# noamteyssier/ibu

Measured on AMD Instinct MI355X. Metric: records/s, fused 2-bit decode+encode of 24-byte IBU records (HBM-resident), higher is better.
Workload: dtype u64

## Files before the change

ibu_amd/csrc/device.cpp:

```cpp
#include <stdlib.h>
#include <stddef.h>
#include <string.h>

#include <chrono>

#include <cstddef>
#include "bgzf_plan.hpp"
#include "ctx.hpp"

using namespace ibu;

namespace {

int32_t check_ctx(const ibu_ctx* ctx) {
  if (!ctx) return err_arg("ctx is NULL");
  hipError_t e = hipSetDevice(ctx->device);
  if (e != hipSuccess) return hip_fail(e, "hipSetDevice");
  return IBU_OK;
}
int32_t check_lens(uint32_t bc_len, uint32_t umi_len) {
  if (bc_len == 0 || bc_len > 32) return err_bc_len(bc_len);
  if (umi_len == 0 || umi_len > 32) return err_umi_len(umi_len);
  return IBU_OK;
}
// ... 131 lines not shown
  if (strcmp(key, "bgzf_range_bytes") == 0) {
    if (value < 0) return err_arg("bgzf_range_bytes must be >= 0");
    ctx->bgzf_range_bytes_opt = (size_t)value;
    return IBU_OK;
  }
  if (strcmp(key, "bgzf_device") == 0) {
    if (value != 0 && value != 1) return err_arg("bgzf_device must be 0 or 1");
    ctx->bgzf_device = (int)value;
    return IBU_OK;
  }
  if (strcmp(key, "bgzf_stream_ahead") == 0) {
    if (value != 0 && value != 1) return err_arg("bgzf_stream_ahead must be 0 or 1");
    ctx->bgzf_stream_ahead = (int)value;
    return IBU_OK;
  }
  if (strcmp(key, "load_piece_delay_ms") == 0) {
    if (value < 0 || value > 10000) return err_arg("load_piece_delay_ms must be 0 .. 10000");
    ctx->load_piece_delay_ms = (uint32_t)value;
    return IBU_OK;
  }
  if (strcmp(key, "release_staging") == 0) {
    if (value != 1) return err_arg("release_staging must be 1");
    if (ctx->stage_lent) return err_arg("an open ibu_stream_open_path stream loads through the staging: close it first");
    IBU_HIP(hipSetDevice(ctx->device));
    for (hipStream_t q : ctx->inflate_streams)
      if (q) IBU_HIP(hipStreamSynchronize(q));
    if (ctx->d_inflate_stage) IBU_HIP(hipFree(ctx->d_inflate_stage));
    ctx->d_inflate_stage = nullptr;
    ctx->inflate_stage_bytes = 0;
    for (int b = 0; b < 2; ++b) {
      if (ctx->d_range_buf[b]) IBU_HIP(hipFree(ctx->d_range_buf[b]));
      ctx->d_range_buf[b] = nullptr;
      ctx->range_buf_bytes[b] = 0;
    }
    return IBU_OK;
  }
  if (strcmp(key, "sort_pull_streams") == 0) {
    if (value != 0 && value != 1) return err_arg("sort_pull_streams must be 0 or 1");
    ctx->force_pull_streams = (int)value;
    return IBU_OK;
  }
  if (strcmp(key, "peer_access") == 0) {
    if (value != 0 && value != 1) return err_arg("peer_access must be 0 or 1");
    ctx->peer_access = (int)value;
    return IBU_OK;
  }
  if (strcmp(key, "numa") == 0) {
    if (value != 0 && value != 1) return err_arg("numa must be 0 (off) or 1 (auto)");
    ctx->numa_mode = (int)value;
    return IBU_OK;
  }
  if (strcmp(key, "trace_rows") == 0) {
    ctx->cfg.trace_rows = value != 0;
    return IBU_OK;
  }
  if (strcmp(key, "base_order") == 0) {
    if (value != IBU_BASE_ORDER_LSB_FIRST && value != IBU_BASE_ORDER_MSB_FIRST) return err_arg("base_order must be 0 (LSB first) or 1 (MSB first)");
    ctx->cfg.base_order = (uint32_t)value;
    return IBU_OK;
  }
  return err_arg("unknown option key");
}
extern "C" int32_t ibu_ctx_device(const ibu_ctx_t* ctx) { return ctx ? ctx->device : -1; }
extern "C" int32_t ibu_ctx_numa(const ibu_ctx_t* ctx, ibu_numa_info_t* out) {
  if (!ctx || !out) return err_arg("ctx or out is NULL");
  memset(out, 0, sizeof *out);
  out->mode = ctx->numa_mode;
  out->node = ctx->place.node;
  out->usable_cpus = ctx->place.ncpus;
  out->ring_node = ctx->ring.slots ? ctx->ring.node : -1;
  out->ring_placed = ctx->ring.slots && ctx->ring.placed ? 1 : 0;
  snprintf(out->pci_bus_id, sizeof out->pci_bus_id, "%s", ctx->pci_bus_id);
  snprintf(out->cpulist, sizeof out->cpulist, "%s", ctx->place.cpulist);
  return IBU_OK;
}
extern "C" void* ibu_ctx_stream(const ibu_ctx_t* ctx) { return ctx ? ctx->stream : nullptr; }
extern "C" int32_t ibu_ctx_synchronize(ibu_ctx_t* ctx, void* stream) {
  int32_t rc = check_ctx(ctx);
  if (rc) return rc;
  IBU_HIP(hipStreamSynchronize(pick_stream(ctx, stream)));
  return IBU_OK;
}
extern "C" int32_t ibu_device_alloc(ibu_ctx_t* ctx, size_t bytes, void** d_ptr) {
  int32_t rc = check_ctx(ctx);
  if (rc) return rc;
  if (!d_ptr) return err_arg("d_ptr is NULL");
  return ibu::ctx_alloc(ctx, bytes, d_ptr);
}
static int32_t alloc_probed_impl(ibu_ctx_t* ctx, size_t bytes, uint32_t tries, void** d_ptr, ibu_alloc_probe_t* report, double alloc_budget_ms,
                                 double* slow_ms);
static uint32_t probe_tries_for(const ibu_ctx* ctx, size_t bytes) {
  const int t = ctx->cfg.alloc_probe_tries;
  if (t == 1) return 1;
  if (t > 1) return bytes >= ((size_t)256 << 20) ? (uint32_t)t : 1u;
  if (bytes < ((size_t)1 << 30)) return 1;
  size_t free_b = 0, total_b = 0;
  if (hipMemGetInfo(&free_b, &total_b) != hipSuccess) { (void)hipGetLastError(); return 1; }
  const size_t fit = free_b / bytes;
  return fit < 3 ? 1u : (fit < 4 ? (uint32_t)fit : 4u);
}
hipError_t ibu::ctx_malloc(ibu_ctx* ctx, void** p, size_t bytes) {
  hipError_t e = hipMalloc(p, bytes ? bytes : 16);
  if (e == hipErrorOutOfMemory && ctx->loser_free.joinable()) {
    (void)hipGetLastError();
    ctx->loser_free.join();
    e = hipMalloc(p, bytes ? bytes : 16);
// ... 849 lines not shown
```

ibu_amd/csrc/k_decode.hip:

```cpp
#include "kcommon.hpp"
#include "kernels.h"

namespace ibu {

constexpr bool dword_len(int len) { return len > 0 && (len & 3) == 0; }
#ifndef IBU_DECODE_GEN_NT
#define IBU_DECODE_GEN_NT 1
#endif
template <int BC, int UM>
constexpr int dec_nt() {
#ifdef IBU_DECODE_NT
  return IBU_DECODE_NT;
#else
  if (BC == 0 && UM == 0) return IBU_DECODE_GEN_NT;
  return (dword_len(BC) && dword_len(UM) && BC + UM >= 20) ? 2 : 1;
#endif
}

template <int NT>
struct DecRegs {
  u32x4 v[3 * NT];
  __device__ __forceinline__ void load(const uint8_t* src) {
#pragma unroll
    for (int k = 0; k < 3 * NT; ++k) v[k] = ld16(src + 1024 * k);
  }
};

template <int BC, int UM, bool MSB>
__device__ __forceinline__ void decode_tile(uint8_t* tile, const DecRegs<dec_nt<BC, UM>()>& a, u32 t, u32 bc_len, u32 umi_len,
                                            uint8_t* bc_out, uint8_t* umi_out, u64* idx_out, u32 lane) {
  constexpr int kDecodeNT = dec_nt<BC, UM>(), kDecLoads = 3 * kDecodeNT, kDecRecs = kTileRecs * kDecodeNT;
  wave_lds_fence();
#pragma unroll
  for (int k = 0; k < kDecLoads; ++k) *reinterpret_cast<u32x4*>(tile + 1024 * k + 16 * lane) = a.v[k];
  wave_lds_fence();
  if constexpr (MSB) {
    rev_pairs_tile<kDecodeNT>(tile, 24, 0, bc_len, lane);
    rev_pairs_tile<kDecodeNT>(tile, 24, 8, umi_len, lane);
    wave_lds_fence();
  }
  u32* const stream_bc = reinterpret_cast<u32*>(tile + kTileBytes * kDecodeNT);
  u32* const stream_umi = reinterpret_cast<u32*>(tile + kTileBytes * kDecodeNT + (BC == 0 ? stream_bytes(kDecodeNT) : 0));
  if (bc_out) expand_field<BC, kDecodeNT>(tile, 24, 0, bc_len, bc_out + (size_t)t * kDecRecs * bc_len, lane, stream_bc);
  if (umi_out) expand_field<UM, kDecodeNT>(tile, 24, 8, umi_len, umi_out + (size_t)t * kDecRecs * umi_len, lane, stream_umi);
  if (idx_out) {
#pragma unroll
    for (int j = 0; j < kDecodeNT; ++j) {
      const u32 c = lane + 64 * j;
      u64 i0 = *reinterpret_cast<const u64*>(tile + (2 * c) * 24 + 16);
      u64 i1 = *reinterpret_cast<const u64*>(tile + (2 * c + 1) * 24 + 16);
      u32x4 o; o.x = (u32)i0; o.y = (u32)(i0 >> 32); o.z = (u32)i1; o.w = (u32)(i1 >> 32);
      st16(reinterpret_cast<uint8_t*>(idx_out) + (size_t)t * (8 * kDecRecs) + 16 * c, o);
    }
  }
}

#ifndef IBU_DECODE_GEN_WAVES
#define IBU_DECODE_GEN_WAVES 6
#endif
template <int BC, int UM, bool MSB>
constexpr int dec_waves() {
  if (BC == 0 || UM == 0) return (BC == 12 || UM == 12) ? 5 : IBU_DECODE_GEN_WAVES;
  if (dec_nt<BC, UM>() > 1) return (BC == 12 || UM == 12) ? 4 : (MSB ? 4 : 5);
  return MSB ? 6 : 7;
}
template <int BC, int UM, bool MSB>
__global__ void __launch_bounds__(kBlock, (dec_waves<BC, UM, MSB>()))
ibu_k_decode(const uint8_t* __restrict__ recs, u32 ntiles, u32 bc_len, u32 umi_len,
             uint8_t* __restrict__ bc_out, uint8_t* __restrict__ umi_out, u64* __restrict__ idx_out) {
  constexpr int kDecBytes = kTileBytes * dec_nt<BC, UM>();
  constexpr int kWaveLds = kDecBytes + ((BC == 0) + (UM == 0)) * (int)stream_bytes(dec_nt<BC, UM>());
  __shared__ __attribute__((aligned(16))) uint8_t lds[kWavesPerBlock * kWaveLds];
  const u32 lane = threadIdx.x & (kWave - 1);
  const u32 wib = threadIdx.x >> 6;
  uint8_t* tile = lds + wib * kWaveLds;
  const TileRange tr = tile_range(ntiles, wib);
  const u32 nwaves = tr.stride;
  u32 t = tr.t;
  ntiles = tr.end;
  if (t >= ntiles) return;
  if (BC > 0) bc_len = BC;
  if (UM > 0) umi_len = UM;

  DecRegs<dec_nt<BC, UM>()> a, b;
  a.load(recs + (size_t)t * kDecBytes + 16 * lane);
  for (;;) {
    u32 tn = t + nwaves;
    bool more = tn < ntiles;
    b.load(recs + (size_t)(more ? tn : t) * kDecBytes + 16 * lane);
    decode_tile<BC, UM, MSB>(tile, a, t, bc_len, umi_len, bc_out, umi_out, idx_out, lane);
    if (!more) break;
    t = tn;
    tn = t + nwaves;
    more = tn < ntiles;
    a.load(recs + (size_t)(more ? tn : t) * kDecBytes + 16 * lane);
    decode_tile<BC, UM, MSB>(tile, b, t, bc_len, umi_len, bc_out, umi_out, idx_out, lane);
    if (!more) break;
    t = tn;
  }
}

#ifndef IBU_UNPACK_GEN_NT
#define IBU_UNPACK_GEN_NT 2
#endif
constexpr int unpack_nt(int len) { return len == 0 ? IBU_UNPACK_GEN_NT : len <= 16 ? 4 : 2; }
constexpr int unpack_waves(int len) { return len == 0 ? 6 : len <= 16 ? 6 : 8; }
template <int LEN, bool MSB>
__global__ void __launch_bounds__(kBlock, unpack_waves(LEN))
ibu_k_unpack(const u64* __restrict__ codes, u32 ntiles , u32 len, uint8_t* __restrict__ out) {
  constexpr int NT = unpack_nt(LEN);
  constexpr int kWaveLds = 1024 * NT + (LEN == 0 ? (int)stream_bytes(NT) : 0);
  __shared__ __attribute__((aligned(16))) uint8_t lds[kWavesPerBlock * kWaveLds];
  const u32 lane = threadIdx.x & (kWave - 1);
  const u32 wib = threadIdx.x >> 6;
  uint8_t* tile = lds + wib * kWaveLds;
  if (LEN > 0) len = LEN;
  const uint8_t* base = reinterpret_cast<const uint8_t*>(codes) + 16 * lane;
  struct Regs { u32x4 v[NT]; };
  sweep_tiles<Regs>(
      tile_range(ntiles, wib),
      [&](Regs& g, u32 t) {
#pragma unroll
        for (int k = 0; k < NT; ++k) g.v[k] = ld16(base + ((size_t)t * NT + k) * 1024);
      },
      [&](const Regs& g, u32 t) {
        wave_lds_fence();
#pragma unroll
        for (int k = 0; k < NT; ++k)
          *reinterpret_cast<u32x4*>(tile + 1024 * k + 16 * lane) = MSB ? rev_pairs_x2(g.v[k], len) : g.v[k];
        wave_lds_fence();
        expand_field<LEN, NT>(tile, 8, 0, len, out + (size_t)t * NT * kTileRecs * len, lane, reinterpret_cast<u32*>(tile + 1024 * NT));
      });
}

__device__ __forceinline__ void unpack_row_bytes(u64 code, u32 len, u32 msb, uint8_t* out) {
  if (msb) code = rev_pairs(code, len);
  for (u32 i = 0; i < len; ++i) {
    const u32 half = (u32)(code >> (i & 16u ? 32 : 0));
    out[i] = (uint8_t)__builtin_amdgcn_ubfe(kPool, 8 * __builtin_amdgcn_ubfe(half, 2 * (i & 15u), 2), 8);
  }
}
extern "C" __global__ void ibu_k_decode_tail(const u64* __restrict__ recs, u64 row0, u64 n, u32 bc_len,
                                             u32 umi_len, u32 msb, uint8_t* bc_out, uint8_t* umi_out, u64* idx_out) {
  const u64 i = row0 + (u64)blockIdx.x * blockDim.x + threadIdx.x;
  if (i >= n) return;
  if (bc_out) unpack_row_bytes(recs[3 * i], bc_len, msb, bc_out + i * bc_len);
  if (umi_out) unpack_row_bytes(recs[3 * i + 1], umi_len, msb, umi_out + i * umi_len);
  if (idx_out) idx_out[i] = recs[3 * i + 2];
}
extern "C" __global__ void ibu_k_unpack_tail(const u64* codes, u64 row0, u64 n, u32 len, u32 msb, uint8_t* out) {
  const u64 i = row0 + (u64)blockIdx.x * blockDim.x + threadIdx.x;
  if (i >= n) return;
  unpack_row_bytes(codes[i], len, msb, out + i * len);
}

typedef void (*DecFn)(const uint8_t*, u32, u32, u32, uint8_t*, uint8_t*, u64*);
template <int B, int U, bool M>
static constexpr DecFn dec_entry() { return ibu_k_decode<len_of_mode(B), len_of_mode(U), M>; }
#define IBU_DEC_ROW(B, M) {dec_entry<B, 0, M>(), dec_entry<B, 1, M>(), dec_entry<B, 2, M>(), dec_entry<B, 3, M>(), dec_entry<B, 4, M>()}
#define IBU_DEC_TABLE(M) {IBU_DEC_ROW(0, M), IBU_DEC_ROW(1, M), IBU_DEC_ROW(2, M), IBU_DEC_ROW(3, M), IBU_DEC_ROW(4, M)}
static const DecFn kDecTable[2][kNumLenModes][kNumLenModes] = {IBU_DEC_TABLE(false), IBU_DEC_TABLE(true)};
template <int B, int U>
static constexpr int dec_recs() { return kTileRecs * dec_nt<len_of_mode(B), len_of_mode(U)>(); }
#define IBU_DEC_RECS_ROW(B) {dec_recs<B, 0>(), dec_recs<B, 1>(), dec_recs<B, 2>(), dec_recs<B, 3>(), dec_recs<B, 4>()}
static const int kDecRecsTable[kNumLenModes][kNumLenModes] = {IBU_DEC_RECS_ROW(0), IBU_DEC_RECS_ROW(1), IBU_DEC_RECS_ROW(2),
                                                              IBU_DEC_RECS_ROW(3), IBU_DEC_RECS_ROW(4)};

hipError_t launch_decode(const LaunchCfg& cfg, const void* recs, size_t n, uint32_t bc_len, uint32_t umi_len,
                         uint8_t* bc, uint8_t* umi, uint64_t* idx, hipStream_t st) {
  (void)hipGetLastError();
  if (n == 0) return hipSuccess;
  const Span sp[4] = {{recs, 24}, {bc, bc_len}, {umi, umi_len}, {idx, 8}};
  const size_t kDecRecs = (size_t)kDecRecsTable[mode_of_len(bc_len)][mode_of_len(umi_len)];
  const RowSplit rs = split_rows(cfg, sp, 4, n, kDecRecs);
  if (rs.head)
    hipLaunchKernelGGL(ibu_k_decode_tail, dim3(tail_grid(rs.head)), dim3(256), 0, st, (const u64*)recs, (u64)0,
                       (u64)rs.head, bc_len, umi_len, cfg.base_order, bc, umi, (u64*)idx);
  if (rs.main) {
    const u32 ntiles = (u32)(rs.main / kDecRecs);
    const int mb = mode_of_len(bc_len), mu = mode_of_len(umi_len);
    const int mo = cfg.base_order ? 1 : 0;
    const DecFn fn = kDecTable[mo][mb][mu];
    static std::atomic<int> occ[2][kNumLenModes][kNumLenModes];
    hipLaunchKernelGGL(fn, dim3(grid_for(ntiles, cfg.cus, resident_blocks<kBlock>(cfg, fn, 0, &occ[mo][mb][mu]))), dim3(kBlock), 0,
                       st, adv((const uint8_t*)recs, 24 * rs.head), ntiles, bc_len, umi_len, adv(bc, rs.head * bc_len),
                       adv(umi, rs.head * umi_len), adv((u64*)idx, 8 * rs.head));
  }
  if (rs.head + rs.main < n)
    hipLaunchKernelGGL(ibu_k_decode_tail, dim3(tail_grid(n - rs.head - rs.main)), dim3(256), 0, st, (const u64*)recs,
                       (u64)(rs.head + rs.main), (u64)n, bc_len, umi_len, cfg.base_order, bc, umi, (u64*)idx);
  return hipGetLastError();
}

typedef void (*UnpFn)(const u64*, u32, u32, uint8_t*);
#define IBU_UNP_ROW(M) {ibu_k_unpack<len_of_mode(0), M>, ibu_k_unpack<len_of_mode(1), M>, ibu_k_unpack<len_of_mode(2), M>, \
                        ibu_k_unpack<len_of_mode(3), M>, ibu_k_unpack<len_of_mode(4), M>}
static const UnpFn kUnpTable[2][kNumLenModes] = {IBU_UNP_ROW(false), IBU_UNP_ROW(true)};

hipError_t launch_unpack(const LaunchCfg& cfg, const uint64_t* codes, size_t n, uint32_t len, uint8_t* out,
                         hipStream_t st) {
  (void)hipGetLastError();
  if (n == 0) return hipSuccess;
  const Span sp[2] = {{codes, 8}, {out, len}};
  const size_t tile_recs = (size_t)kTileRecs * unpack_nt(len_of_mode(mode_of_len(len)));
  const RowSplit rs = split_rows(cfg, sp, 2, n, tile_recs);
  if (rs.head)
    hipLaunchKernelGGL(ibu_k_unpack_tail, dim3(tail_grid(rs.head)), dim3(256), 0, st, (const u64*)codes, (u64)0, (u64)rs.head,
                       len, cfg.base_order, out);
  if (rs.main) {
    const u32 ntiles = (u32)(rs.main / tile_recs);
    const int m = mode_of_len(len), mo = cfg.base_order ? 1 : 0;
    static std::atomic<int> occ[2][kNumLenModes];
    hipLaunchKernelGGL(kUnpTable[mo][m], dim3(grid_for(ntiles, cfg.cus, resident_blocks<kBlock>(cfg, kUnpTable[mo][m], 0, &occ[mo][m]))),
                       dim3(kBlock), 0, st, adv((const u64*)codes, 8 * rs.head), ntiles, len, adv(out, rs.head * len));
  }
  if (rs.head + rs.main < n)
    hipLaunchKernelGGL(ibu_k_unpack_tail, dim3(tail_grid(n - rs.head - rs.main)), dim3(256), 0, st, (const u64*)codes,
                       (u64)(rs.head + rs.main), (u64)n, len, cfg.base_order, out);
  return hipGetLastError();
}

}
```

ibu_amd/csrc/k_encode.hip:

```cpp
#include "kcommon.hpp"
#include "kernels.h"

namespace ibu {

#ifndef IBU_ENCODE_MINWAVES
#define IBU_ENCODE_MINWAVES 6
#endif
#ifndef IBU_ENCODE_GEN_MINWAVES
#define IBU_ENCODE_GEN_MINWAVES 4
#endif
constexpr int encode_minwaves(int bc, int um) {
  if (bc == 0 || um == 0) return IBU_ENCODE_GEN_MINWAVES;
  return (bc <= 16 && um <= 16) ? IBU_ENCODE_MINWAVES : 4;
}
__host__ __device__ constexpr u32 enc_field_lds(int spec_len, u32 len) { return spec_len > 0 ? 128u * len : 32u * len + kStreamPad; }
template <int BC, int UM>
constexpr int enc_nt() {
#ifdef IBU_ENCODE_NT
  return (BC > 0 && UM > 0 && (BC & 3) == 0 && (UM & 3) == 0) ? IBU_ENCODE_NT : 1;
#else
  return 1;
#endif
}
#ifndef IBU_ENCODE_NT2_MINWAVES
#define IBU_ENCODE_NT2_MINWAVES 5
#endif
template <int BC, int UM>
constexpr int enc_waves() { return enc_nt<BC, UM>() > 1 ? IBU_ENCODE_NT2_MINWAVES : encode_minwaves(BC, UM); }

template <int BC, int UM, bool MSB>
__global__ void __launch_bounds__(kBlock, (enc_waves<BC, UM>()))
ibu_k_encode(const uint8_t* __restrict__ bc_in, const uint8_t* __restrict__ umi_in,
             const u64* __restrict__ idx_in, u64 first_index, u64 row_base, u32 ntiles, u32 bc_len, u32 umi_len,
             u32 wave_lds_bytes, uint8_t* __restrict__ recs, u64* __restrict__ status) {
  constexpr int NT = enc_nt<BC, UM>(), kRecs = kTileRecs * NT;
  extern __shared__ __attribute__((aligned(16))) uint8_t dyn_lds[];
  const u32 lane = threadIdx.x & (kWave - 1);
  const u32 wib = threadIdx.x >> 6;
  if (BC > 0) bc_len = BC;
  if (UM > 0) umi_len = UM;
  uint8_t* area = dyn_lds + wib * wave_lds_bytes;
  uint8_t* asc_bc = area;
  uint8_t* asc_umi = area + enc_field_lds(BC, bc_len) * NT;
  const TileRange tr = tile_range(ntiles, wib);
  const u32 nwaves = tr.stride;
  u32 t = tr.t;
  ntiles = tr.end;
  if (t >= ntiles) return;
  const uint8_t* idx_src = idx_in ? reinterpret_cast<const uint8_t*>(idx_in) + 16 * lane : bc_in;
  const size_t idx_tile = idx_in ? 1024 * NT : 0, idx_sub = idx_in ? 1024 : 0;

  AsciiStage<BC, NT> sb;
  AsciiStage<UM, NT> su;
  u32x4 vi[NT];
  sb.issue(bc_in + (size_t)t * kRecs * bc_len, bc_len, lane);
  su.issue(umi_in + (size_t)t * kRecs * umi_len, umi_len, lane);
#pragma unroll
  for (int j = 0; j < NT; ++j) vi[j] = ld16(idx_src + (size_t)t * idx_tile + j * idx_sub);
  BadRows bad;
  for (;;) {
    const size_t row0 = (size_t)t * kRecs;
    wave_lds_fence();
    const bool okcb = sb.land(asc_bc, bc_len, lane), okcu = su.land(asc_umi, umi_len, lane);
    const bool chunks_ok = okcb && okcu;
    u64 ix[NT][2];
#pragma unroll
    for (int j = 0; j < NT; ++j) {
      ix[j][0] = ((u64)vi[j].y << 32) | vi[j].x;
      ix[j][1] = ((u64)vi[j].w << 32) | vi[j].z;
      if (!idx_in) { ix[j][0] = first_index + row0 + 128 * j + 2 * lane; ix[j][1] = ix[j][0] + 1; }
    }
    const u32 tn = t + nwaves;
    const bool more = tn < ntiles;
    const u32 tp = more ? tn : t;
    sb.issue(bc_in + (size_t)tp * kRecs * bc_len, bc_len, lane);
    su.issue(umi_in + (size_t)tp * kRecs * umi_len, umi_len, lane);
#pragma unroll
    for (int j = 0; j < NT; ++j) vi[j] = ld16(idx_src + (size_t)tp * idx_tile + j * idx_sub);
    wave_lds_fence();
    u64 b[NT][2], u[NT][2];
#pragma unroll
    for (int j = 0; j < NT; ++j)
#pragma unroll
      for (int h = 0; h < 2; ++h) {
        const u32 r = 128 * j + 2 * lane + h;
        bool okb = true, oku = true;
#if IBU_PROBE == 1
        b[j][h] = *reinterpret_cast<const u32*>(asc_bc + r * bc_len);
        u[j][h] = *reinterpret_cast<const u32*>(asc_umi + r * umi_len);
#elif IBU_PROBE == 2
        b[j][h] = row0 + r;
        u[j][h] = b[j][h] * 3;
#else
        b[j][h] = pack_row<BC>(asc_bc, r, bc_len, okb);
        u[j][h] = pack_row<UM>(asc_umi, r, umi_len, oku);
        if constexpr (BC == 0 || UM == 0) {
          if (__ballot(!chunks_ok) != 0) {
            if constexpr (BC == 0) b[j][h] = pack_row_bytes(bc_in + (row0 + r) * bc_len, bc_len, okb);
            if constexpr (UM == 0) u[j][h] = pack_row_bytes(umi_in + (row0 + r) * umi_len, umi_len, oku);
          }
        }
#endif
        if (!okb) b[j][h] = 0;
        if (!oku) u[j][h] = 0;
        bad.note(!(okb && oku), row_base + row0 + r);
      }
    wave_lds_fence();
#pragma unroll
    for (int j = 0; j < NT; ++j) {
      u64* r = reinterpret_cast<u64*>(area + (128 * j + 2 * lane) * 24);
      r[0] = b[j][0]; r[1] = u[j][0]; r[2] = ix[j][0]; r[3] = b[j][1]; r[4] = u[j][1]; r[5] = ix[j][1];
    }
    wave_lds_fence();
    if constexpr (MSB) {
      rev_pairs_tile<NT>(area, 24, 0, bc_len, lane);
      rev_pairs_tile<NT>(area, 24, 8, umi_len, lane);
      wave_lds_fence();
    }
    uint8_t* dst = recs + (size_t)t * (kTileBytes * NT) + 16 * lane;
#pragma unroll
    for (int k = 0; k < 3 * NT; ++k) st16(dst + 1024 * k, *reinterpret_cast<const u32x4*>(area + 1024 * k + 16 * lane));
    if (!more) break;
    t = tn;
  }
  bad.flush(status);
}

constexpr int pack_nt(int len) { return (len > 0 && len <= 16) ? 2 : 1; }
template <int LEN, bool MSB, int GNT = 1, int RND = 0>
__global__ void __launch_bounds__(kBlock, LEN == 0 ? (RND >= 7 ? 5 : (GNT >= 4 || RND >= 5) ? 6 : 8) : LEN <= 12 ? 5 : 4)
ibu_k_pack(const uint8_t* __restrict__ in, u64 row_base, u32 ntiles , u32 len, u64* __restrict__ codes,
           u64* __restrict__ status) {
  constexpr int NT = LEN > 0 ? pack_nt(LEN) : GNT, kRows = kTileRecs * NT;
  constexpr u32 kWaveLds = LEN > 0 ? (u32)(kRows * LEN) : (u32)(256 * (RND > 0 ? RND : 4)) + kStreamPad;
  __shared__ __attribute__((aligned(16))) uint8_t lds[kWavesPerBlock * kWaveLds];
  const u32 lane = threadIdx.x & (kWave - 1);
  const u32 wib = threadIdx.x >> 6;
  uint8_t* asc = lds + wib * kWaveLds;
  const TileRange tr = tile_range(ntiles, wib);
  const u32 nwaves = tr.stride;
  u32 t = tr.t;
  ntiles = tr.end;
  if (LEN > 0) len = LEN;
  if (t >= ntiles) return;
  AsciiStage<LEN, NT, RND> sv;
  sv.issue(in + (size_t)t * kRows * len, len, lane);
  BadRows bad;
  for (;;) {
    const size_t row0 = (size_t)t * kRows;
    wave_lds_fence();
    const bool chunks_ok = sv.land(asc, len, lane);
    const u32 tn = t + nwaves;
    const bool more = tn < ntiles;
    sv.issue(in + (size_t)(more ? tn : t) * kRows * len, len, lane);
    wave_lds_fence();
#pragma unroll
    for (int j = 0; j < NT; ++j) {
      const u32 r = 128 * j + 2 * lane;
      bool ok0 = true, ok1 = true;
      u64 v0 = pack_row<LEN>(asc, r, len, ok0);
      u64 v1 = pack_row<LEN>(asc, r + 1, len, ok1);
      if constexpr (LEN == 0) {
        if (__ballot(!chunks_ok) != 0) {
          v0 = pack_row_bytes(in + (row0 + r) * len, len, ok0);
          v1 = pack_row_bytes(in + (row0 + r + 1) * len, len, ok1);
        }
      }
      if constexpr (MSB) { v0 = rev_pairs(v0, len); v1 = rev_pairs(v1, len); }
      if (!ok0) v0 = 0;
      if (!ok1) v1 = 0;
      bad.note(!ok0, row_base + row0 + r);
      bad.note(!ok1, row_base + row0 + r + 1);
      u32x4 o; o.x = (u32)v0; o.y = (u32)(v0 >> 32); o.z = (u32)v1; o.w = (u32)(v1 >> 32);
      st16(reinterpret_cast<uint8_t*>(codes) + (row0 + 128 * j) * 8 + 16 * lane, o);
    }
    if (!more) break;
    t = tn;
  }
  bad.flush(status);
}

extern "C" __global__ void ibu_k_encode_tail(const uint8_t* bc_in, const uint8_t* umi_in, const u64* idx_in,
                                             u64 first_index, u64 row0, u64 n, u32 bc_len, u32 umi_len, u32 msb,
                                             u64* __restrict__ recs, u64* status) {
  const u64 i = row0 + (u64)blockIdx.x * blockDim.x + threadIdx.x;
  if (i >= n) return;
  bool okb = true, oku = true;
  u64 b = pack_row_bytes(bc_in + i * bc_len, bc_len, okb);
  u64 u = pack_row_bytes(umi_in + i * umi_len, umi_len, oku);
  if (msb) { b = rev_pairs(b, bc_len); u = rev_pairs(u, umi_len); }
  if (!okb) b = 0;
  if (!oku) u = 0;
  if (!(okb && oku)) { atomicMin(&status[0], i); atomicAdd(&status[1], 1ull); }
  recs[3 * i] = b; recs[3 * i + 1] = u; recs[3 * i + 2] = idx_in ? idx_in[i] : first_index + i;
}
extern "C" __global__ void ibu_k_pack_tail(const uint8_t* in, u64 row0, u64 n, u32 len, u32 msb, u64* codes, u64* status) {
  const u64 i = row0 + (u64)blockIdx.x * blockDim.x + threadIdx.x;
  if (i >= n) return;
  bool ok = true;
  u64 v = pack_row_bytes(in + i * len, len, ok);
  if (msb) v = rev_pairs(v, len);
  if (!ok) { v = 0; atomicMin(&status[0], i); atomicAdd(&status[1], 1ull); }
  codes[i] = v;
}

typedef void (*EncFn)(const uint8_t*, const uint8_t*, const u64*, u64, u64, u32, u32, u32, u32, uint8_t*, u64*);
template <int B, int U, bool M>
static constexpr EncFn enc_entry() { return ibu_k_encode<len_of_mode(B), len_of_mode(U), M>; }
#define IBU_ENC_ROW(B, M) {enc_entry<B, 0, M>(), enc_entry<B, 1, M>(), enc_entry<B, 2, M>(), enc_entry<B, 3, M>(), enc_entry<B, 4, M>()}
#define IBU_ENC_TABLE(M) {IBU_ENC_ROW(0, M), IBU_ENC_ROW(1, M), IBU_ENC_ROW(2, M), IBU_ENC_ROW(3, M), IBU_ENC_ROW(4, M)}
static const EncFn kEncTable[2][kNumLenModes][kNumLenModes] = {IBU_ENC_TABLE(false), IBU_ENC_TABLE(true)};
template <int B, int U>
static constexpr int enc_nt_of() { return enc_nt<len_of_mode(B), len_of_mode(U)>(); }
#define IBU_ENC_NT_ROW(B) {enc_nt_of<B, 0>(), enc_nt_of<B, 1>(), enc_nt_of<B, 2>(), enc_nt_of<B, 3>(), enc_nt_of<B, 4>()}
static const int kEncNtTable[kNumLenModes][kNumLenModes] = {IBU_ENC_NT_ROW(0), IBU_ENC_NT_ROW(1), IBU_ENC_NT_ROW(2),
                                                            IBU_ENC_NT_ROW(3), IBU_ENC_NT_ROW(4)};

hipError_t launch_encode(const LaunchCfg& cfg, const uint8_t* bc, const uint8_t* umi, const uint64_t* idx,
                         uint64_t first_index, size_t n, uint32_t bc_len, uint32_t umi_len, void* recs,
                         uint64_t* status, hipStream_t st) {
  (void)hipGetLastError();
  if (n == 0) return hipSuccess;
  const Span sp[4] = {{recs, 24}, {bc, bc_len}, {umi, umi_len}, {idx, 8}};
  const int mb = mode_of_len(bc_len), mu = mode_of_len(umi_len);
  const u32 nt = (u32)kEncNtTable[mb][mu];
  const size_t tile_recs = (size_t)kTileRecs * nt;
  const RowSplit rs = split_rows(cfg, sp, 4, n, tile_recs);
  if (rs.head)
    hipLaunchKernelGGL(ibu_k_encode_tail, dim3(tail_grid(rs.head)), dim3(256), 0, st, bc, umi, (const u64*)idx, (u64)first_index,
                       (u64)0, (u64)rs.head, bc_len, umi_len, cfg.base_order, (u64*)recs, (u64*)status);
  if (rs.main) {
    const u32 ntiles = (u32)(rs.main / tile_recs);
    u32 wave_lds = (enc_field_lds(len_of_mode(mb), bc_len) + enc_field_lds(len_of_mode(mu), umi_len)) * nt;
    if (wave_lds < (u32)kTileBytes * nt) wave_lds = kTileBytes * nt;
    const int mo = cfg.base_order ? 1 : 0;
    const EncFn fn = kEncTable[mo][mb][mu];
    static std::atomic<int> occ[2][33][33];
    const int nb = resident_blocks<kBlock>(cfg, fn, wave_lds * kWavesPerBlock, &occ[mo][bc_len][umi_len]);
    hipLaunchKernelGGL(fn, dim3(grid_for(ntiles, cfg.cus, nb)), dim3(kBlock), wave_lds * kWavesPerBlock, st,
                       adv(bc, rs.head * bc_len), adv(umi, rs.head * umi_len), adv((const u64*)idx, 8 * rs.head),
                       (u64)(first_index + rs.head), (u64)rs.head, ntiles, bc_len, umi_len, wave_lds,
                       adv((uint8_t*)recs, 24 * rs.head), (u64*)status);
  }
  if (rs.head + rs.main < n)
    hipLaunchKernelGGL(ibu_k_encode_tail, dim3(tail_grid(n - rs.head - rs.main)), dim3(256), 0, st, bc, umi, (const u64*)idx,
                       (u64)first_index, (u64)(rs.head + rs.main), (u64)n, bc_len, umi_len, cfg.base_order, (u64*)recs, (u64*)status);
  return hipGetLastError();
}

typedef void (*PackFn)(const uint8_t*, u64, u32, u32, u64*, u64*);
#define IBU_PACK_ROW(M) {nullptr , ibu_k_pack<len_of_mode(1), M>, ibu_k_pack<len_of_mode(2), M>, \
                         ibu_k_pack<len_of_mode(3), M>, ibu_k_pack<len_of_mode(4), M>}
static const PackFn kPackTable[2][kNumLenModes] = {IBU_PACK_ROW(false), IBU_PACK_ROW(true)};
struct PackShape { int nt, rounds; };
static inline PackShape pack_shape(uint32_t len) {
  const int nt = len <= 8 ? 4 : 2;
  return {nt, (int)(len * nt + 7) / 8};
}
template <bool M>
static PackFn pack_gen_entry(int nt, int rounds) {
  switch (nt * 10 + rounds) {
    case 41: return ibu_k_pack<0, M, 4, 1>;
    case 42: return ibu_k_pack<0, M, 4, 2>;
    case 43: return ibu_k_pack<0, M, 4, 3>;
    case 44: return ibu_k_pack<0, M, 4, 4>;
    case 23: return ibu_k_pack<0, M, 2, 3>;
    case 24: return ibu_k_pack<0, M, 2, 4>;
    case 25: return ibu_k_pack<0, M, 2, 5>;
    case 26: return ibu_k_pack<0, M, 2, 6>;
    case 27: return ibu_k_pack<0, M, 2, 7>;
    default: return ibu_k_pack<0, M, 2, 8>;
  }
}

hipError_t launch_pack(const LaunchCfg& cfg, const uint8_t* in, size_t n, uint32_t len, uint64_t* codes,
                       uint64_t* status, hipStream_t st) {
  (void)hipGetLastError();
  if (n == 0) return hipSuccess;
  const Span sp[2] = {{in, len}, {codes, 8}};
  const int m = mode_of_len(len), mo = cfg.base_order ? 1 : 0;
  const PackShape shape = m ? PackShape{pack_nt(len_of_mode(m)), 0} : pack_shape(len);
  const size_t tile_rows = (size_t)kTileRecs * shape.nt;
  const RowSplit rs = split_rows(cfg, sp, 2, n, tile_rows);
  if (rs.head)
    hipLaunchKernelGGL(ibu_k_pack_tail, dim3(tail_grid(rs.head)), dim3(256), 0, st, in, (u64)0, (u64)rs.head, len, cfg.base_order,
                       (u64*)codes, (u64*)status);
  if (rs.main) {
    const u32 ntiles = (u32)(rs.main / tile_rows);
    const PackFn fn = m ? kPackTable[mo][m] : (mo ? pack_gen_entry<true>(shape.nt, shape.rounds) : pack_gen_entry<false>(shape.nt, shape.rounds));
    static std::atomic<int> occ[2][kNumLenModes], occ_gen[2][33];
    std::atomic<int>* oc = m ? &occ[mo][m] : &occ_gen[mo][len];
    hipLaunchKernelGGL(fn, dim3(grid_for(ntiles, cfg.cus, resident_blocks<kBlock>(cfg, fn, 0, oc))),
                       dim3(kBlock), 0, st, adv(in, rs.head * len), (u64)rs.head, ntiles, len, adv((u64*)codes, 8 * rs.head),
                       (u64*)status);
  }
// ... 8 lines not shown
```

ibu_amd/csrc/kcommon.hpp:

```cpp
#pragma once
#include <hip/hip_runtime.h>
#include <stdint.h>
#include <stdio.h>
#include <stdlib.h>

#include "kernels.h"

namespace ibu {

typedef unsigned int u32;
typedef unsigned long long u64;
typedef u32 u32x4 __attribute__((ext_vector_type(4)));
typedef u32 u32x2 __attribute__((ext_vector_type(2)));

static constexpr int kWave = 64;
#ifndef IBU_BLOCK
#define IBU_BLOCK 256
#endif
static constexpr int kBlock = IBU_BLOCK;
static constexpr int kWavesPerBlock = kBlock / kWave;
static constexpr int kTileRecs = 128;
static constexpr int kTileBytes = kTileRecs * 24;
static constexpr u32 kPool = 0x54474341u;

static constexpr int kNumLenModes = 5;
__host__ __device__ constexpr int len_of_mode(int m) { return m == 1 ? 8 : m == 2 ? 12 : m == 3 ? 16 : m == 4 ? 32 : 0; }
static inline int mode_of_len(uint32_t len) {
  switch (len) {
    case 8: return 1;
    case 12: return 2;
    case 16: return 3;
    case 32: return 4;
    default: return 0;
  }
}

#ifndef IBU_XCD_REMAP
#define IBU_XCD_REMAP 1
#endif
__device__ __forceinline__ u32 logical_block() {
#if IBU_XCD_REMAP
  const u32 nb = gridDim.x;
  if (nb & 7u) return blockIdx.x;
  return (blockIdx.x & 7u) * (nb >> 3) + (blockIdx.x >> 3);
#else
  return blockIdx.x;
#endif
}

#ifndef IBU_XCD_STATIC
#define IBU_XCD_STATIC 1
#endif
struct TileRange { u32 t, stride, end; };
#ifndef IBU_XCD_SUB
#define IBU_XCD_SUB 1
#endif
__device__ __forceinline__ TileRange tile_range(u32 ntiles, u32 wib) {
#if IBU_XCD_STATIC
  if ((gridDim.x & 7u) == 0 && gridDim.x >= 8u * IBU_XCD_SUB) {
    const u32 parts = 8u * IBU_XCD_SUB;
    const u32 tpp = (ntiles + parts - 1) / parts;
    const u32 xcd = blockIdx.x & 7u, lb = blockIdx.x >> 3, nbx = gridDim.x >> 3;
    const u32 sub = lb % IBU_XCD_SUB, part = xcd * IBU_XCD_SUB + sub;
    const u32 nb_sub = (nbx - sub + IBU_XCD_SUB - 1) / IBU_XCD_SUB;
    const u32 t0 = part * tpp, t1 = t0 + tpp < ntiles ? t0 + tpp : ntiles;
    return {t0 + (lb / IBU_XCD_SUB) * (u32)kWavesPerBlock + wib, nb_sub * (u32)kWavesPerBlock, t0 < ntiles ? t1 : 0u};
  }
#endif
  return {logical_block() * (u32)kWavesPerBlock + wib, gridDim.x * (u32)kWavesPerBlock, ntiles};
}

template <class Regs, class Load, class Body>
__device__ __forceinline__ void sweep_tiles(const TileRange tr, Load load, Body body) {
  u32 t = tr.t;
  if (t >= tr.end) return;
  Regs a, b;
  load(a, t);
  for (;;) {
    u32 tn = t + tr.stride;
    bool more = tn < tr.end;
    load(b, more ? tn : t);
    body(a, t);
    if (!more) break;
    t = tn;
    tn = t + tr.stride;
    more = tn < tr.end;
    load(a, more ? tn : t);
    body(b, t);
    if (!more) break;
    t = tn;
  }
}

#ifndef IBU_NT_LOAD
#define IBU_NT_LOAD 1
#endif
#ifndef IBU_NT_STORE
#define IBU_NT_STORE 1
#endif
#ifndef IBU_ST_POLICY
#define IBU_ST_POLICY 0
#endif
#ifndef IBU_LD_POLICY
#define IBU_LD_POLICY 0
#endif
struct WaveBuf {
  __amdgpu_buffer_rsrc_t r;
  u32 voff;
  __device__ __forceinline__ explicit WaveBuf(const void* p) {
    const u64 a = (u64)p;
    const u64 first = ((u64)(u32)__builtin_amdgcn_readfirstlane((u32)(a >> 32)) << 32) | (u64)(u32)__builtin_amdgcn_readfirstlane((u32)a);
    const u64 base = first - (1ull << 30);
    r = __builtin_amdgcn_make_buffer_rsrc(reinterpret_cast<void*>(base), 0, -1, 0x00020000);
    voff = (u32)(a - base);
  }
};
__device__ __forceinline__ u32x4 ld16(const void* p) {
#if IBU_LD_POLICY
  const WaveBuf w(p);
  return __builtin_amdgcn_raw_buffer_load_b128(w.r, (int)w.voff, 0, IBU_LD_POLICY - 1);
#elif IBU_NT_LOAD
  return __builtin_nontemporal_load(reinterpret_cast<const u32x4*>(p));
// ... 204 lines not shown
    for (int i = 0; i < rounds; ++i) {
      u32 c = lane + 64 * i;
      c = c < last ? c : last;
      v[i] = ld16(g + 16 * (size_t)c);
    }
  }
  __device__ __forceinline__ bool land(uint8_t* lds, u32 rt_len, u32 lane) const {
    const u32 nchunks = 8 * (LEN > 0 ? (u32)(LEN * NT) : rt_len * NT);
    bool ok = true;
#pragma unroll
    for (int i = 0; i < rounds; ++i) {
      const u32 c = lane + 64 * i;
      if constexpr (LEN > 0) {
        if (c < nchunks) *reinterpret_cast<u32x4*>(lds + 16 * c) = v[i];
      } else {
        if (64u * i < nchunks) {
          bool okc = true;
          const u32 w = pack4(v[i].x, okc) | (pack4(v[i].y, okc) << 8) | (pack4(v[i].z, okc) << 16) | (pack4(v[i].w, okc) << 24);
          if (c < nchunks) { reinterpret_cast<u32*>(lds)[c] = w; ok = ok && okc; }
        }
      }
    }
    return ok;
  }
};

struct BadRows {
  u64 first = ~0ull;
  u32 count = 0;
  __device__ __forceinline__ void note(bool bad, u64 row_global) {
    if (bad) { first = row_global < first ? row_global : first; ++count; }
  }
  __device__ __forceinline__ void flush(u64* status) const {
    if (__ballot(count != 0) == 0) return;
    u64 f = first;
    u32 c = count;
#pragma unroll
    for (int m = 32; m >= 1; m >>= 1) {
      const u32 flo = __shfl_xor((u32)f, m), fhi = __shfl_xor((u32)(f >> 32), m);
      const u64 fo = ((u64)fhi << 32) | flo;
      f = fo < f ? fo : f;
      c += __shfl_xor(c, m);
    }
    if ((threadIdx.x & (kWave - 1)) == 0) { atomicMin(&status[0], f); atomicAdd(&status[1], (u64)c); }
  }
};


static inline u32 grid_for(u32 ntiles, int cus, int blocks_per_cu) {
  u32 need = (ntiles + kWavesPerBlock - 1) / kWavesPerBlock;
  u32 cap = (u32)(cus * blocks_per_cu);
  return need < cap ? (need ? need : 1) : cap;
}
static inline bool aligned16(const void* p) { return (reinterpret_cast<uintptr_t>(p) & 15u) == 0; }

struct Span { const void* p; size_t stride; };
static inline int peel_rows(const Span* s, int k) {
  for (int h = 0; h < 16; ++h) {
    bool ok = true;
    for (int i = 0; i < k; ++i)
      if (s[i].p && ((reinterpret_cast<uintptr_t>(s[i].p) + (uintptr_t)h * s[i].stride) & 15u)) ok = false;
    if (ok) return h;
  }
  return -1;
}
struct RowSplit { size_t head, main; };
static inline RowSplit split_rows(const LaunchCfg& cfg, const Span* s, int k, size_t n, size_t tile) {
  const int h = peel_rows(s, k);
  RowSplit rs{n, 0};
  if (h >= 0) {
    rs.head = (size_t)h < n ? (size_t)h : n;
    rs.main = ((n - rs.head) / tile) * tile;
  }
  if (cfg.trace_rows) fprintf(stderr, "ibu rows: n=%zu head=%zu tiled=%zu rest=%zu tile=%zu\n", n, rs.head, rs.main, n - rs.head - rs.main, tile);
  return rs;
}
template <class T> static inline T* adv(T* p, size_t bytes) {
  return p ? reinterpret_cast<T*>(reinterpret_cast<uintptr_t>(p) + bytes) : p;
}
static inline u32 tail_grid(u64 rows) { return (u32)((rows + 255) / 256); }
static inline u32 capped_grid(const LaunchCfg& cfg, u64 items, u64 per_block, u32 blocks_per_cu = 8) {
  u64 blocks = (items + per_block - 1) / per_block;
  const u64 cap = (u64)cfg.cus * blocks_per_cu;
  if (blocks > cap) blocks = cap;
  return (u32)(blocks ? blocks : 1);
}

__device__ __forceinline__ u64 shfl_xor64(u64 v, int m) {
  u32 lo = __shfl_xor((u32)v, m), hi = __shfl_xor((u32)(v >> 32), m);
  return ((u64)hi << 32) | lo;
}
__device__ __forceinline__ u64 shfl_up64(u64 v, int d) {
  u32 lo = __shfl_up((u32)v, d), hi = __shfl_up((u32)(v >> 32), d);
  return ((u64)hi << 32) | lo;
}
__device__ __forceinline__ u32 shfl_xor_lanes(u32 v, int m) { return __shfl_xor(v, m); }
__device__ __forceinline__ u64 shfl_xor_lanes(u64 v, int m) { return shfl_xor64(v, m); }
__device__ __forceinline__ u32 shfl_up_lanes(u32 v, int d) { return __shfl_up(v, d); }
__device__ __forceinline__ u64 shfl_up_lanes(u64 v, int d) { return shfl_up64(v, d); }
struct OpAdd { template <class T> __device__ __forceinline__ T operator()(T a, T b) const { return a + b; } };
struct OpMin { template <class T> __device__ __forceinline__ T operator()(T a, T b) const { return b < a ? b : a; } };
template <class T, class Op>
__device__ __forceinline__ T wave_reduce(T v, Op op) {
#pragma unroll
  for (int m = 32; m >= 1; m >>= 1) v = op(v, shfl_xor_lanes(v, m));
  return v;
// ... 38 lines not shown
```

ibu_amd/csrc/kernels.h:

```cpp
#pragma once
#include <hip/hip_runtime.h>
#include <stddef.h>
#include <stdint.h>

#include <atomic>

namespace ibu {

struct LaunchCfg {
  int cus = 256;
  int blocks_per_cu = 7;
  int sort_variant = 0;
  int sort_guess = 1;
  int sort_compact = 1;
  int sort_hybrid = 1;
  int sort_idx64 = 0;
  int alloc_probe_tries = 0;
  int trace_rows = 0;
  uint32_t base_order = 0;
};

template <int BLOCK, class K>
static inline int resident_blocks(const LaunchCfg& cfg, K kernel, size_t dyn_lds, std::atomic<int>* cache) {
  int cached = cache->load(std::memory_order_relaxed);
  if (cached <= 0) {
    int nb = 0;
    if (hipOccupancyMaxActiveBlocksPerMultiprocessor(&nb, kernel, BLOCK, dyn_lds) != hipSuccess || nb <= 0)
      nb = 1024 / BLOCK;
    cache->store(nb, std::memory_order_relaxed);
    cached = nb;
  }
  int cap = cfg.blocks_per_cu * 256 / BLOCK;
  if (cap < 1) cap = 1;
  return cached < cap ? cached : cap;
}

hipError_t launch_decode(const LaunchCfg&, const void* recs, size_t n, uint32_t bc_len, uint32_t umi_len,
                         uint8_t* bc, uint8_t* umi, uint64_t* idx, hipStream_t st);
hipError_t launch_encode(const LaunchCfg&, const uint8_t* bc, const uint8_t* umi, const uint64_t* idx,
                         uint64_t first_index, size_t n, uint32_t bc_len, uint32_t umi_len, void* recs,
                         uint64_t* status, hipStream_t st);
hipError_t launch_deserialize(const LaunchCfg&, const void* recs, size_t n, uint64_t* bc, uint64_t* umi,
                              uint64_t* idx, hipStream_t st);
hipError_t launch_serialize(const LaunchCfg&, const uint64_t* bc, const uint64_t* umi, const uint64_t* idx,
                            size_t n, void* recs, hipStream_t st);
hipError_t launch_unpack(const LaunchCfg&, const uint64_t* codes, size_t n, uint32_t len, uint8_t* out,
                         hipStream_t st);
hipError_t launch_pack(const LaunchCfg&, const uint8_t* in, size_t n, uint32_t len, uint64_t* codes,
                       uint64_t* status, hipStream_t st);
static constexpr int kReduceSlots = 64;
static constexpr size_t kReduceAccBytes = (size_t)kReduceSlots * 8 * sizeof(uint64_t);
hipError_t launch_reduce(const LaunchCfg&, const void* recs, size_t n, uint64_t* acc, hipStream_t st);
hipError_t launch_reduce_fold(uint64_t* acc, hipStream_t st);
hipError_t launch_generate(const LaunchCfg&, uint64_t seed, uint64_t first, size_t n, uint32_t bc_len,
                           uint32_t umi_len, void* recs, hipStream_t st);
hipError_t launch_copy(const LaunchCfg&, const void* src, void* dst, size_t bytes, hipStream_t st);
hipError_t launch_sorted_check(const LaunchCfg&, const void* recs, size_t n, uint32_t* flag, hipStream_t st);
hipError_t launch_mismatch(const LaunchCfg&, const void* a, const void* b, size_t nwords, uint64_t* first, hipStream_t st);
hipError_t launch_fill2(uint64_t* p, uint64_t v0, uint64_t v1, hipStream_t st);

bool trace_sort();
hipError_t launch_sort_records(const LaunchCfg&, void* recs, void* tmp, size_t n, void* scratch,
                               size_t scratch_bytes, hipStream_t st, const uint64_t* known_words = nullptr ,
                               int known_prefix = -1 );
size_t sort_scratch_bytes(const LaunchCfg&, size_t n);
size_t sort_prefix_estimate_tables(const LaunchCfg&, size_t n);
int sort_num_variants();
int sort_num_compact_variants();
hipError_t launch_lower_bound(const void* recs, size_t n, const void* keys, size_t k, uint64_t* pos, hipStream_t st);
struct CompactPlan {
  uint32_t csel[4][3];
// ... 97 lines not shown
```

Before: 51.26 billion.

## Add optional interleaved XCD segment tile mapping for decode and encode kernels

Measured after the change: 50.90 billion. About the same (-0.7%).

```diff
diff --git a/ibu_amd/csrc/device.cpp b/ibu_amd/csrc/device.cpp
--- a/ibu_amd/csrc/device.cpp
+++ b/ibu_amd/csrc/device.cpp
@@ -207,6 +207,11 @@
   }
   if (strcmp(key, "trace_rows") == 0) {
     ctx->cfg.trace_rows = value != 0;
+    return IBU_OK;
+  }
+  if (strcmp(key, "xcd_segment_records_log2") == 0) {
+    if (value != 0 && (value < 7 || value > 32)) return err_arg("xcd_segment_records_log2 must be 0 (contiguous eighths) or 7 .. 32");
+    ctx->cfg.xcd_segment_records_log2 = (int)value;
     return IBU_OK;
   }
   if (strcmp(key, "base_order") == 0) {
diff --git a/ibu_amd/csrc/k_decode.hip b/ibu_amd/csrc/k_decode.hip
--- a/ibu_amd/csrc/k_decode.hip
+++ b/ibu_amd/csrc/k_decode.hip
@@ -67,14 +67,14 @@
 template <int BC, int UM, bool MSB>
 __global__ void __launch_bounds__(kBlock, (dec_waves<BC, UM, MSB>()))
 ibu_k_decode(const uint8_t* __restrict__ recs, u32 ntiles, u32 bc_len, u32 umi_len,
-             uint8_t* __restrict__ bc_out, uint8_t* __restrict__ umi_out, u64* __restrict__ idx_out) {
+             uint8_t* __restrict__ bc_out, uint8_t* __restrict__ umi_out, u64* __restrict__ idx_out, u32 seg_k) {
   constexpr int kDecBytes = kTileBytes * dec_nt<BC, UM>();
   constexpr int kWaveLds = kDecBytes + ((BC == 0) + (UM == 0)) * (int)stream_bytes(dec_nt<BC, UM>());
   __shared__ __attribute__((aligned(16))) uint8_t lds[kWavesPerBlock * kWaveLds];
   const u32 lane = threadIdx.x & (kWave - 1);
-  const u32 wib = threadIdx.x >> 6;
+  const u32 wib = (u32)__builtin_amdgcn_readfirstlane((int)(threadIdx.x >> 6));
   uint8_t* tile = lds + wib * kWaveLds;
-  const TileRange tr = tile_range(ntiles, wib);
+  const TileRange tr = tile_range(ntiles, wib, seg_k);
   const u32 nwaves = tr.stride;
   u32 t = tr.t;
   ntiles = tr.end;
@@ -83,18 +83,18 @@
   if (UM > 0) umi_len = UM;
 
   DecRegs<dec_nt<BC, UM>()> a, b;
-  a.load(recs + (size_t)t * kDecBytes + 16 * lane);
+  a.load(recs + (size_t)tile_at(tr, t) * kDecBytes + 16 * lane);
   for (;;) {
     u32 tn = t + nwaves;
     bool more = tn < ntiles;
-    b.load(recs + (size_t)(more ? tn : t) * kDecBytes + 16 * lane);
-    decode_tile<BC, UM, MSB>(tile, a, t, bc_len, umi_len, bc_out, umi_out, idx_out, lane);
+    b.load(recs + (size_t)tile_at(tr, more ? tn : t) * kDecBytes + 16 * lane);
+    decode_tile<BC, UM, MSB>(tile, a, tile_at(tr, t), bc_len, umi_len, bc_out, umi_out, idx_out, lane);
     if (!more) break;
     t = tn;
     tn = t + nwaves;
     more = tn < ntiles;
-    a.load(recs + (size_t)(more ? tn : t) * kDecBytes + 16 * lane);
-    decode_tile<BC, UM, MSB>(tile, b, t, bc_len, umi_len, bc_out, umi_out, idx_out, lane);
+    a.load(recs + (size_t)tile_at(tr, more ? tn : t) * kDecBytes + 16 * lane);
+    decode_tile<BC, UM, MSB>(tile, b, tile_at(tr, t), bc_len, umi_len, bc_out, umi_out, idx_out, lane);
     if (!more) break;
     t = tn;
   }
@@ -154,7 +154,7 @@
   unpack_row_bytes(codes[i], len, msb, out + i * len);
 }
 
-typedef void (*DecFn)(const uint8_t*, u32, u32, u32, uint8_t*, uint8_t*, u64*);
+typedef void (*DecFn)(const uint8_t*, u32, u32, u32, uint8_t*, uint8_t*, u64*, u32);
 template <int B, int U, bool M>
 static constexpr DecFn dec_entry() { return ibu_k_decode<len_of_mode(B), len_of_mode(U), M>; }
 #define IBU_DEC_ROW(B, M) {dec_entry<B, 0, M>(), dec_entry<B, 1, M>(), dec_entry<B, 2, M>(), dec_entry<B, 3, M>(), dec_entry<B, 4, M>()}
@@ -184,7 +184,7 @@
     static std::atomic<int> occ[2][kNumLenModes][kNumLenModes];
     hipLaunchKernelGGL(fn, dim3(grid_for(ntiles, cfg.cus, resident_blocks<kBlock>(cfg, fn, 0, &occ[mo][mb][mu]))), dim3(kBlock), 0,
                        st, adv((const uint8_t*)recs, 24 * rs.head), ntiles, bc_len, umi_len, adv(bc, rs.head * bc_len),
-                       adv(umi, rs.head * umi_len), adv((u64*)idx, 8 * rs.head));
+                       adv(umi, rs.head * umi_len), adv((u64*)idx, 8 * rs.head), xcd_segment_k(cfg, kDecRecs));
   }
   if (rs.head + rs.main < n)
     hipLaunchKernelGGL(ibu_k_decode_tail, dim3(tail_grid(n - rs.head - rs.main)), dim3(256), 0, st, (const u64*)recs,
diff --git a/ibu_amd/csrc/k_encode.hip b/ibu_amd/csrc/k_encode.hip
--- a/ibu_amd/csrc/k_encode.hip
+++ b/ibu_amd/csrc/k_encode.hip
@@ -32,17 +32,17 @@
 __global__ void __launch_bounds__(kBlock, (enc_waves<BC, UM>()))
 ibu_k_encode(const uint8_t* __restrict__ bc_in, const uint8_t* __restrict__ umi_in,
              const u64* __restrict__ idx_in, u64 first_index, u64 row_base, u32 ntiles, u32 bc_len, u32 umi_len,
-             u32 wave_lds_bytes, uint8_t* __restrict__ recs, u64* __restrict__ status) {
+             u32 wave_lds_bytes, uint8_t* __restrict__ recs, u64* __restrict__ status, u32 seg_k) {
   constexpr int NT = enc_nt<BC, UM>(), kRecs = kTileRecs * NT;
   extern __shared__ __attribute__((aligned(16))) uint8_t dyn_lds[];
   const u32 lane = threadIdx.x & (kWave - 1);
-  const u32 wib = threadIdx.x >> 6;
+  const u32 wib = (u32)__builtin_amdgcn_readfirstlane((int)(threadIdx.x >> 6));
   if (BC > 0) bc_len = BC;
   if (UM > 0) umi_len = UM;
   uint8_t* area = dyn_lds + wib * wave_lds_bytes;
   uint8_t* asc_bc = area;
   uint8_t* asc_umi = area + enc_field_lds(BC, bc_len) * NT;
-  const TileRange tr = tile_range(ntiles, wib);
+  const TileRange tr = tile_range(ntiles, wib, seg_k);
   const u32 nwaves = tr.stride;
   u32 t = tr.t;
   ntiles = tr.end;
@@ -53,13 +53,15 @@
   AsciiStage<BC, NT> sb;
   AsciiStage<UM, NT> su;
   u32x4 vi[NT];
-  sb.issue(bc_in + (size_t)t * kRecs * bc_len, bc_len, lane);
-  su.issue(umi_in + (size_t)t * kRecs * umi_len, umi_len, lane);
-#pragma unroll
-  for (int j = 0; j < NT; ++j) vi[j] = ld16(idx_src + (size_t)t * idx_tile + j * idx_sub);
+  const u32 p0 = tile_at(tr, t);
+  sb.issue(bc_in + (size_t)p0 * kRecs * bc_len, bc_len, lane);
+  su.issue(umi_in + (size_t)p0 * kRecs * umi_len, umi_len, lane);
+#pragma unroll
+  for (int j = 0; j < NT; ++j) vi[j] = ld16(idx_src + (size_t)p0 * idx_tile + j * idx_sub);
   BadRows bad;
   for (;;) {
-    const size_t row0 = (size_t)t * kRecs;
+    const u32 pt = tile_at(tr, t);
+    const size_t row0 = (size_t)pt * kRecs;
     wave_lds_fence();
     const bool okcb = sb.land(asc_bc, bc_len, lane), okcu = su.land(asc_umi, umi_len, lane);
     const bool chunks_ok = okcb && okcu;
@@ -72,7 +74,7 @@
     }
     const u32 tn = t + nwaves;
     const bool more = tn < ntiles;
-    const u32 tp = more ? tn : t;
+    const u32 tp = tile_at(tr, more ? tn : t);
     sb.issue(bc_in + (size_t)tp * kRecs * bc_len, bc_len, lane);
     su.issue(umi_in + (size_t)tp * kRecs * umi_len, umi_len, lane);
 #pragma unroll
@@ -117,7 +119,7 @@
       rev_pairs_tile<NT>(area, 24, 8, umi_len, lane);
       wave_lds_fence();
     }
-    uint8_t* dst = recs + (size_t)t * (kTileBytes * NT) + 16 * lane;
+    uint8_t* dst = recs + (size_t)pt * (kTileBytes * NT) + 16 * lane;
 #pragma unroll
     for (int k = 0; k < 3 * NT; ++k) st16(dst + 1024 * k, *reinterpret_cast<const u32x4*>(area + 1024 * k + 16 * lane));
     if (!more) break;
@@ -204,7 +206,7 @@
   codes[i] = v;
 }
 
-typedef void (*EncFn)(const uint8_t*, const uint8_t*, const u64*, u64, u64, u32, u32, u32, u32, uint8_t*, u64*);
+typedef void (*EncFn)(const uint8_t*, const uint8_t*, const u64*, u64, u64, u32, u32, u32, u32, uint8_t*, u64*, u32);
 template <int B, int U, bool M>
 static constexpr EncFn enc_entry() { return ibu_k_encode<len_of_mode(B), len_of_mode(U), M>; }
 #define IBU_ENC_ROW(B, M) {enc_entry<B, 0, M>(), enc_entry<B, 1, M>(), enc_entry<B, 2, M>(), enc_entry<B, 3, M>(), enc_entry<B, 4, M>()}
@@ -240,7 +242,7 @@
     hipLaunchKernelGGL(fn, dim3(grid_for(ntiles, cfg.cus, nb)), dim3(kBlock), wave_lds * kWavesPerBlock, st,
                        adv(bc, rs.head * bc_len), adv(umi, rs.head * umi_len), adv((const u64*)idx, 8 * rs.head),
                        (u64)(first_index + rs.head), (u64)rs.head, ntiles, bc_len, umi_len, wave_lds,
-                       adv((uint8_t*)recs, 24 * rs.head), (u64*)status);
+                       adv((uint8_t*)recs, 24 * rs.head), (u64*)status, xcd_segment_k(cfg, tile_recs));
   }
   if (rs.head + rs.main < n)
     hipLaunchKernelGGL(ibu_k_encode_tail, dim3(tail_grid(n - rs.head - rs.main)), dim3(256), 0, st, bc, umi, (const u64*)idx,
diff --git a/ibu_amd/csrc/kcommon.hpp b/ibu_amd/csrc/kcommon.hpp
--- a/ibu_amd/csrc/kcommon.hpp
+++ b/ibu_amd/csrc/kcommon.hpp
@@ -51,23 +51,41 @@
 #ifndef IBU_XCD_STATIC
 #define IBU_XCD_STATIC 1
 #endif
-struct TileRange { u32 t, stride, end; };
 #ifndef IBU_XCD_SUB
 #define IBU_XCD_SUB 1
 #endif
-__device__ __forceinline__ TileRange tile_range(u32 ntiles, u32 wib) {
+struct TileRange { u32 t, stride, end, seg_base = 0, seg_end = 0, seg_x = 0, seg_shift = 0; };
+__host__ __device__ __forceinline__ u32 tile_at(const TileRange& tr, u32 l) {
+  const u32 j = l - tr.seg_base, s = tr.seg_shift;
+  const u32 p = ((j >> s) << (s + 3)) + tr.seg_x + (j & ((1u << s) - 1u));
+  return l < tr.seg_end ? p : l;
+}
+__host__ __device__ __forceinline__ TileRange tile_range_of(u32 ntiles, u32 nblocks, u32 block, u32 wib, u32 k = 0) {
 #if IBU_XCD_STATIC
-  if ((gridDim.x & 7u) == 0 && gridDim.x >= 8u * IBU_XCD_SUB) {
+  if ((nblocks & 7u) == 0 && nblocks >= 8u * IBU_XCD_SUB) {
+    const u32 s = (k && IBU_XCD_SUB == 1) ? k - 1 : 0;
+    const u32 gf = (k && IBU_XCD_SUB == 1) ? (ntiles >> (s + 3)) << s : 0u;
+    const u32 rest0 = gf << 3, rest = ntiles - rest0;
     const u32 parts = 8u * IBU_XCD_SUB;
-    const u32 tpp = (ntiles + parts - 1) / parts;
-    const u32 xcd = blockIdx.x & 7u, lb = blockIdx.x >> 3, nbx = gridDim.x >> 3;
+    const u32 tpp = (rest + parts - 1) / parts;
+    const u32 xcd = block & 7u, lb = block >> 3, nbx = nblocks >> 3;
     const u32 sub = lb % IBU_XCD_SUB, part = xcd * IBU_XCD_SUB + sub;
     const u32 nb_sub = (nbx - sub + IBU_XCD_SUB - 1) / IBU_XCD_SUB;
-    const u32 t0 = part * tpp, t1 = t0 + tpp < ntiles ? t0 + tpp : ntiles;
-    return {t0 + (lb / IBU_XCD_SUB) * (u32)kWavesPerBlock + wib, nb_sub * (u32)kWavesPerBlock, t0 < ntiles ? t1 : 0u};
-  }
-#endif
-  return {logical_block() * (u32)kWavesPerBlock + wib, gridDim.x * (u32)kWavesPerBlock, ntiles};
+    const u32 t0 = rest0 + part * tpp, t1 = t0 + tpp < ntiles ? t0 + tpp : ntiles;
+    const u32 base = t0 - gf;
+    return {base + (lb / IBU_XCD_SUB) * (u32)kWavesPerBlock + wib, nb_sub * (u32)kWavesPerBlock, t0 < ntiles ? t1 : (gf ? t0 : 0u),
+            base, gf ? t0 : 0u, xcd << s, s};
+  }
+#endif
+#if IBU_XCD_REMAP
+  const u32 lblock = (nblocks & 7u) ? block : (block & 7u) * (nblocks >> 3) + (block >> 3);
+#else
+  const u32 lblock = block;
+#endif
+  return {lblock * (u32)kWavesPerBlock + wib, nblocks * (u32)kWavesPerBlock, ntiles, 0u, 0u, 0u, 0u};
+}
+__device__ __forceinline__ TileRange tile_range(u32 ntiles, u32 wib, u32 k = 0) {
+  return tile_range_of(ntiles, gridDim.x, blockIdx.x, wib, k);
 }
 
 template <class Regs, class Load, class Body>
@@ -378,6 +396,13 @@
   u32 cap = (u32)(cus * blocks_per_cu);
   return need < cap ? (need ? need : 1) : cap;
 }
+static inline u32 xcd_segment_k(const LaunchCfg& cfg, size_t tile_recs) {
+  if (cfg.xcd_segment_records_log2 <= 0) return 0;
+  int tile_log2 = 0;
+  while (((size_t)1 << (tile_log2 + 1)) <= tile_recs) ++tile_log2;
+  const int g = cfg.xcd_segment_records_log2 - tile_log2;
+  return (u32)(g < 0 ? 0 : g > 28 ? 28 : g) + 1;
+}
 static inline bool aligned16(const void* p) { return (reinterpret_cast<uintptr_t>(p) & 15u) == 0; }
 
 struct Span { const void* p; size_t stride; };
diff --git a/ibu_amd/csrc/kernels.h b/ibu_amd/csrc/kernels.h
--- a/ibu_amd/csrc/kernels.h
+++ b/ibu_amd/csrc/kernels.h
@@ -17,6 +17,7 @@
   int sort_idx64 = 0;
   int alloc_probe_tries = 0;
   int trace_rows = 0;
+  int xcd_segment_records_log2 = 0;
   uint32_t base_order = 0;
 };
 
```
